# cv-stuttgart/PCFA

Measured on AMD Instinct MI355X. Metric: attack_steps_per_sec, higher is better.
Workload: dtype f32; 1 GPU; RAFT, 1 synthetic 436x1024 pair per GPU (padded 440x1024), disjoint delta, change_of_variables, delta_bound=0.005, zero target, L-BFGS max_iter=10; weights=random:1234, parallelism=pairs sharded 1/GPU, closure_launch=hipGraph replay

## Files before the change

### include/pcfa_hip.h

```cpp
#ifndef PCFA_HIP_H
#define PCFA_HIP_H

#include <stddef.h>
#include <stdint.h>

#ifdef __cplusplus
extern "C" {
#endif

#define PCFA_OK 0
#define PCFA_ERR_INVALID_ARG (-1)
#define PCFA_ERR_UNSUPPORTED (-2)
#define PCFA_ERR_WORKSPACE (-3)

#if defined(__GNUC__)
#define PCFA_API __attribute__((visibility("default")))
#else
#define PCFA_API
#endif

#define PCFA_MAX_LEVELS 8
#define PCFA_ABI_VERSION 2

#define PCFA_LOSS_AEE 0
#define PCFA_LOSS_MSE 1
#define PCFA_LOSS_COSIM 2

#define PCFA_BOX_CLIPPING 0
#define PCFA_BOX_CHANGE_OF_VARIABLES 1

PCFA_API int pcfa_abi_version(void);
PCFA_API int pcfa_timing_arm(void* start_event, void* stop_event, int nth);

PCFA_API int pcfa_null_launch(void* stream);
PCFA_API int pcfa_poison_lds(unsigned pattern, void* stream);
PCFA_API int pcfa_peek_lds(unsigned* out, int n, void* stream);
PCFA_API long long pcfa_calib_mfma_f32(float* scratch, int blocks, int iters, void* stream);
PCFA_API int pcfa_calib_copy(const float* src, float* dst, long long n_floats, void* stream);
PCFA_API const char* pcfa_status_string(int status);


PCFA_API long long pcfa_corr_slab_floats(int H, int W, int num_levels);
PCFA_API long long pcfa_corr_level_offset(int H, int W, int num_levels, int level, int* h_l, int* w_l);

PCFA_API long long pcfa_corr_tiled_index(int H, int W, int num_levels, int level, int y, int x);

PCFA_API int pcfa_corr_f2ext_fwd(const float* fmap2, float* f2ext, int B, int D, int H, int W,
                        int num_levels, void* stream);

PCFA_API int pcfa_corr_pyramid_fwd(const float* fmap1, const float* f2ext, float* pyr, int B, int D,
                          int H, int W, int num_levels, void* stream);

PCFA_API size_t pcfa_corr_pyramid_bwd_workspace_bytes(int B, int D, int H, int W, int num_levels);
PCFA_API int pcfa_corr_pyramid_bwd(const float* dpyr, const float* fmap1, const float* f2ext,
                          float* dfmap1, float* dfmap2, void* workspace, size_t workspace_bytes,
                          int B, int D, int H, int W, int num_levels, void* stream);
PCFA_API size_t pcfa_corr_pyramid_bwd_windows_workspace_bytes(int B, int D, int H, int W, int num_levels);
PCFA_API int pcfa_corr_pyramid_bwd_windows(const float* dpyr, const float* fmap1, const float* f2ext, float* dfmap1,
                                  float* dfmap2, void* workspace, size_t workspace_bytes,
                                  const float* const* coords, int n_coords, int radius, int B, int D, int H, int W,
                                  int num_levels, void* stream);

PCFA_API int pcfa_corr_lookup_fwd(const float* pyr, const float* coords, float* out, int B, int H, int W,
                         int num_levels, int radius, void* stream);

PCFA_API int pcfa_corr_lookup_bwd(float* dpyr, const float* coords, const float* grad_out, int B, int H,
                         int W, int num_levels, int radius, void* stream);

PCFA_API size_t pcfa_corr_ondemand_workspace_bytes(int B, int D, int H, int W, int num_levels);
PCFA_API int pcfa_corr_ondemand_prepare(const float* fmap1, const float* fmap2, void* workspace, int B, int D, int H,
                               int W, int num_levels, void* stream);
PCFA_API int pcfa_corr_ondemand_fwd(const void* workspace, const float* coords, float* out, int B, int D, int H, int W,
                           int num_levels, int radius, void* stream);
PCFA_API int pcfa_corr_ondemand_bwd(void* workspace, const float* coords, const float* grad_out, int accumulate, int B,
                           int D, int H, int W, int num_levels, int radius, void* stream);
PCFA_API int pcfa_corr_ondemand_finish(const void* workspace, float* dfmap1, float* dfmap2, int B, int D, int H, int W,
                              int num_levels, void* stream);

PCFA_API int pcfa_corr_ondemand_fwd_tiled(const void* workspace, const float* coords, float* out, int B, int D, int H,
                                 int W, int num_levels, int radius, void* stream);
PCFA_API int pcfa_corr_ondemand_bwd_tiled(void* workspace, const float* coords, const float* grad_out, int accumulate,
                                 int B, int D, int H, int W, int num_levels, int radius, void* stream);
PCFA_API int pcfa_corr_ondemand_tile_geometry(int* tile_w, int* tile_h, int* max_positions);
PCFA_API int pcfa_corr_ondemand_tile_routes(const void* workspace, int B, int D, int H, int W, int num_levels,
                                   int* counts, void* stream);

PCFA_API size_t pcfa_gemm_f32_workspace_bytes(int M, int N, int batch, int splits);
PCFA_API int pcfa_gemm_f32(const float* A, const float* B, float* C, int M, int N, int K, long long lda, long long ldb,
                  long long ldc, int a_kmajor, int b_kmajor, int batch, long long bsA, long long bsB, long long bsC,
                  float alpha, int splits, void* workspace, size_t workspace_bytes, void* stream);
// ... 330 lines not shown
```

### pcfa_amd/_hip.py

```python
import ctypes
import os
from ctypes import c_char_p, c_double, c_float, c_int, c_longlong, c_size_t, c_uint, c_void_p, POINTER

ABI_VERSION = 2
LIB_PATH = os.environ.get("PCFA_HIP_LIB") or os.path.join(os.path.dirname(os.path.abspath(__file__)), "lib",
                                                          "libpcfa_hip.so")

PCFA_LOSS = {"aee": 0, "mse": 1, "cosim": 2}


class HipLibraryError(RuntimeError):
    pass


_P = c_void_p
_S4 = POINTER(c_longlong)

SIGNATURES = {
    "pcfa_abi_version": (c_int, []),
    "pcfa_timing_arm": (c_int, [_P, _P, c_int]),
    "pcfa_null_launch": (c_int, [_P]),
    "pcfa_poison_lds": (c_int, [c_uint, _P]),
    "pcfa_peek_lds": (c_int, [_P, c_int, _P]),
    "pcfa_calib_mfma_f32": (c_longlong, [_P, c_int, c_int, _P]),
    "pcfa_calib_copy": (c_int, [_P, _P, c_longlong, _P]),
    "pcfa_status_string": (c_char_p, [c_int]),
    "pcfa_corr_slab_floats": (c_longlong, [c_int, c_int, c_int]),
    "pcfa_corr_level_offset": (c_longlong, [c_int, c_int, c_int, c_int, POINTER(c_int), POINTER(c_int)]),
    "pcfa_corr_tiled_index": (c_longlong, [c_int, c_int, c_int, c_int, c_int, c_int]),
    "pcfa_corr_f2ext_fwd": (c_int, [_P, _P, c_int, c_int, c_int, c_int, c_int, _P]),
    "pcfa_corr_pyramid_fwd": (c_int, [_P, _P, _P, c_int, c_int, c_int, c_int, c_int, _P]),
    "pcfa_corr_pyramid_bwd_workspace_bytes": (c_size_t, [c_int, c_int, c_int, c_int, c_int]),
    "pcfa_corr_pyramid_bwd": (c_int, [_P, _P, _P, _P, _P, _P, c_size_t, c_int, c_int, c_int, c_int, c_int, _P]),
    "pcfa_corr_pyramid_bwd_windows_workspace_bytes": (c_size_t, [c_int, c_int, c_int, c_int, c_int]),
    "pcfa_corr_pyramid_bwd_windows": (c_int, [_P, _P, _P, _P, _P, _P, c_size_t, POINTER(c_void_p), c_int, c_int, c_int,
                                              c_int, c_int, c_int, c_int, _P]),
    "pcfa_corr_lookup_fwd": (c_int, [_P, _P, _P, c_int, c_int, c_int, c_int, c_int, _P]),
    "pcfa_corr_lookup_bwd": (c_int, [_P, _P, _P, c_int, c_int, c_int, c_int, c_int, _P]),
    "pcfa_corr_ondemand_workspace_bytes": (c_size_t, [c_int, c_int, c_int, c_int, c_int]),
    "pcfa_corr_ondemand_prepare": (c_int, [_P, _P, _P, c_int, c_int, c_int, c_int, c_int, _P]),
    "pcfa_corr_ondemand_fwd": (c_int, [_P, _P, _P, c_int, c_int, c_int, c_int, c_int, c_int, _P]),
    "pcfa_corr_ondemand_bwd": (c_int, [_P, _P, _P, c_int, c_int, c_int, c_int, c_int, c_int, c_int, _P]),
    "pcfa_corr_ondemand_finish": (c_int, [_P, _P, _P, c_int, c_int, c_int, c_int, c_int, _P]),
    "pcfa_corr_ondemand_fwd_tiled": (c_int, [_P, _P, _P, c_int, c_int, c_int, c_int, c_int, c_int, _P]),
    "pcfa_corr_ondemand_bwd_tiled": (c_int, [_P, _P, _P, c_int, c_int, c_int, c_int, c_int, c_int, c_int, _P]),
    "pcfa_corr_ondemand_tile_geometry": (c_int, [POINTER(c_int), POINTER(c_int), POINTER(c_int)]),
    "pcfa_corr_ondemand_tile_routes": (c_int, [_P, c_int, c_int, c_int, c_int, c_int, _P, _P]),
    "pcfa_gemm_f32_workspace_bytes": (c_size_t, [c_int, c_int, c_int, c_int]),
    "pcfa_gemm_f32": (c_int, [_P, _P, _P, c_int, c_int, c_int, c_longlong, c_longlong, c_longlong, c_int, c_int, c_int,
                              c_longlong, c_longlong, c_longlong, c_float, c_int, _P, c_size_t, _P]),
    "pcfa_gemm_bf16x3_workspace_bytes": (c_size_t, [c_int, c_int, c_int, c_int]),
    "pcfa_gemm_bf16x3": (c_int, [_P, _P, _P, c_int, c_int, c_int, c_longlong, c_longlong, c_longlong, c_int, c_int,
                                 c_int, c_longlong, c_longlong, c_longlong, c_float, c_int, _P, c_size_t, _P]),
    "pcfa_corr_pyramid_fwd_bf16x3": (c_int, [_P, _P, _P, c_int, c_int, c_int, c_int, c_int, _P]),
    "pcfa_softmax_rows_fwd": (c_int, [_P, _P, c_longlong, c_int, _P]),
    "pcfa_softmax_rows_bwd": (c_int, [_P, _P, _P, c_longlong, c_int, _P]),
    "pcfa_attn_stream_lse": (c_int, [_P, _P, _P, c_int, c_int, c_int, c_float, _P]),
    "pcfa_attn_stream_fwd": (c_int, [_P, _P, _P, _P, _P, c_int, c_int, c_int, c_float, _P]),
    "pcfa_attn_stream_dv": (c_int, [_P, _P, _P, _P, _P, c_int, c_int, c_int, c_float, _P]),
    "pcfa_attn_stream_delta": (c_int, [_P, _P, _P, c_longlong, c_int, c_int, _P]),
    "pcfa_attn_stream_dqk": (c_int, [_P, _P, _P, _P, _P, _P, _P, _P, c_int, c_int, c_int, c_int, c_float, _P]),
    "pcfa_lookup_convc1_packed_floats": (c_longlong, [c_int]),
    "pcfa_lookup_convc1_pack_weights": (c_int, [_P, _P, c_int, c_int, _P]),
    "pcfa_lookup_convc1_fwd": (c_int, [_P, _P, _P, _P, _P, c_int, c_int, c_int, c_int, c_int, c_int, c_int, _P]),
    "pcfa_lookup_convc1_bwd": (c_int, [_P, _P, _P, _P, _P, c_int, c_int, c_int, c_int, c_int, c_int, c_int, _P]),
    "pcfa_spatial_corr_out_size": (c_int, [c_int] * 10 + [POINTER(c_int), POINTER(c_int)]),
    "pcfa_spatial_corr_fwd": (c_int, [_P, _P, _P] + [c_int] * 16 + [_P]),
# ... 182 lines not shown
```

### pcfa_amd/csrc/corr_pyramid.hip

```cpp
#include "common.hpp"
#include "gemm_tile.hpp"

namespace {

#ifndef PCFA_GEMM_BK
#define PCFA_GEMM_BK 16
#endif
#ifndef PCFA_GEMM_STORE_MID
#define PCFA_GEMM_STORE_MID 0
#endif
#ifndef PCFA_GEMM_STORE_MID_AT
#define PCFA_GEMM_STORE_MID_AT 4
#endif
constexpr int BK = PCFA_GEMM_BK;
constexpr int NLD = BK / 8;
constexpr int KV = BK / 4;
constexpr int LDS_KM = 132;
constexpr int LDS_MK = 130;

template <bool KMAJ>
__device__ __forceinline__ void tile_load(const float* __restrict__ X, long long ld, int dim,
                                          int d0, int k0, int kend, bool vec, float4 (&r)[NLD]) {
  const int tid = threadIdx.x;
#pragma unroll
// ... 109 lines not shown
      row + (okY ? u.off1 + (((Y1 >> 2) * u.tw1 + (X1 >> 2)) << 4) + ((Y1 & 3) << 2) + (X1 & 3) : 0));
  const float d1a = (okY && X1 < u.w1) ? g1.x + 0.25f * d2 : 0.f;
  const float d1b = (okY && X1 + 1 < u.w1) ? g1.y + 0.25f * d2 : 0.f;
  v.x += 0.25f * d1a;
  v.y += 0.25f * d1a;
  v.z += 0.25f * d1b;
  v.w += 0.25f * d1b;
  return v;
}

template <bool KMAJ>
__device__ __forceinline__ void tile_load_unpool(const float* __restrict__ X, long long ld, int dim, int d0, int k0,
                                                 int kend, const UnpoolArgs& u, float4 (&r)[NLD]) {
  static_assert(BK % 16 == 0, "whole 4x4 tiles per stage and query");
  const int tid = threadIdx.x;
#pragma unroll
  for (int i = 0; i < NLD; ++i) {
    const int f = tid + 256 * i;
    int q, col;
    if (KMAJ) {
      q = min(k0 + f / 32, kend - 1);
      col = min(d0 + (f % 32) * 4, dim - 4);
    } else {
      q = min(d0 + f / KV, dim - 1);
      col = min(k0 + (f % KV) * 4, kend - 4);
    }
    const int T0 = col >> 4, y = (col & 15) >> 2;
    const int ty = T0 / u.tw0, tx = T0 - ty * u.tw0;
    const float* row = X + (long long)q * ld;
    r[i] = unpool_piece(row, *reinterpret_cast<const float4*>(row + col), ty, tx, y, u);
  }
}

constexpr int SEG_INTS = 10;
template <bool A_KM, bool B_KN, bool FAST, bool POOL, bool UNPOOL = false, bool SPARSE = false>
__device__ __forceinline__ void gemm_f32_mfma_body(
    const float* __restrict__ A, const float* __restrict__ B, float* __restrict__ C, int M,
    int N, int K, long long lda, long long ldb, long long ldc, long long bsA, long long bsB,
    long long bsC, int splits, int kchunk, long long ssC, float div, int vecA, int vecB, const PoolArgs& pool,
    const UnpoolArgs& unpool = UnpoolArgs{}, const int* __restrict__ segs = nullptr) {
  static_assert(!UNPOOL || FAST, "the un-pooling loader is the branch-free one");
  static_assert(!SPARSE || (FAST && !POOL && !UNPOOL), "segment lists ride on the branch-free loader");
  constexpr int SA = A_KM ? LDS_KM : LDS_MK;
  constexpr int SB = B_KN ? LDS_KM : LDS_MK;
  constexpr int STAGE = 2 * BK * SA + 2 * BK * SB;
  constexpr int LDSF = POOL && BM * SC > STAGE ? BM * SC : STAGE;
  __shared__ __attribute__((aligned(16))) float smem[LDSF];
  float (*sA)[BK * SA] = reinterpret_cast<float (*)[BK * SA]>(smem);
  float (*sB)[BK * SB] = reinterpret_cast<float (*)[BK * SB]>(smem + 2 * BK * SA);

  const int batch = blockIdx.z / splits;
  const int split = blockIdx.z - batch * splits;
  A += batch * bsA;
  B += batch * bsB;
  C += batch * bsC + split * ssC;
  int kbeg = split * kchunk;
  const int kend = SPARSE ? K : min(K, kbeg + kchunk);
  int by = blockIdx.y, bx = blockIdx.x;
  gemm_tile_xcd_order(by, bx);
  const int m0 = by * BM;
  int n0 = bx * BN;
  bool pooled = false;
  if (POOL) {
    if (bx < pool.nb0) {
      pooled = true;
      N = pool.S0;
    } else {
      n0 = pool.off_tail + (bx - pool.nb0) * BN;
    }
  }

  const int lane = threadIdx.x & 63, wave = threadIdx.x >> 6;
  const int wr = wave >> 1, wc = wave & 1;
  const int l31 = lane & 31, lh = lane >> 5;

  f32x16 acc[2][2];
#pragma unroll
  for (int i = 0; i < 2; ++i)
#pragma unroll
    for (int j = 0; j < 2; ++j)
#pragma unroll
      for (int r = 0; r < 16; ++r) acc[i][j][r] = 0.f;

  float4 ra[NLD], rb[NLD];
  int nk = (kend - kbeg + BK - 1) / BK;
  int sb[4] = {0, 0, 0, 0}, se[4] = {0, 0, 0, 0}, seg = 0;
  if (SPARSE) {
    const int* sg = segs + ((long long)batch * gridDim.x + bx) * SEG_INTS;
    int total = 0;
#pragma unroll
    for (int i = 0; i < 4; ++i) {
      sb[i] = sg[1 + 2 * i];
      se[i] = sg[2 + 2 * i];
      total += (se[i] - sb[i]) / BK;
    }
    const int t0 = (int)((long long)total * split / splits), t1 = (int)((long long)total * (split + 1) / splits);
    nk = t1 - t0;
    int rem = t0;
    while (seg < 3 && rem >= (se[seg] - sb[seg]) / BK) {
      rem -= (se[seg] - sb[seg]) / BK;
      ++seg;
    }
    kbeg = sb[seg] + rem * BK;
  }
  int kcur = kbeg;
  if (nk > 0) {
    if (FAST) {
      tile_load_fast<A_KM>(A, lda, M, m0, kbeg, kend, ra);
      if (UNPOOL) tile_load_unpool<B_KN>(B, ldb, N, n0, kbeg, kend, unpool, rb);
      else tile_load_fast<B_KN>(B, ldb, N, n0, kbeg, kend, rb);
      tile_mask<A_KM>(M, m0, kbeg, kend, ra);
      tile_mask<B_KN>(N, n0, kbeg, kend, rb);
    } else {
      tile_load<A_KM>(A, lda, M, m0, kbeg, kend, vecA, ra);
      tile_load<B_KN>(B, ldb, N, n0, kbeg, kend, vecB, rb);
    }
    tile_store<A_KM>(sA[0], ra);
    tile_store<B_KN>(sB[0], rb);
  }
  __syncthreads();
  int cur = 0;
  for (int kt = 0; kt < nk; ++kt) {
    const bool more = kt + 1 < nk;
    int k0 = kbeg + (kt + 1) * BK;
    if (SPARSE) {
      k0 = kcur + BK;
      if (k0 >= se[seg] && seg < 3 && se[seg + 1] > sb[seg + 1]) {
        ++seg;
        k0 = sb[seg];
      }
      kcur = k0;
    }
    if (FAST) {
      tile_load_fast<A_KM>(A, lda, M, m0, min(k0, kend - 4), kend, ra);
      if (UNPOOL) tile_load_unpool<B_KN>(B, ldb, N, n0, min(k0, kend - 4), kend, unpool, rb);
      else tile_load_fast<B_KN>(B, ldb, N, n0, min(k0, kend - 4), kend, rb);
      __builtin_amdgcn_sched_barrier(0);
    } else if (more) {
      tile_load<A_KM>(A, lda, M, m0, k0, kend, vecA, ra);
      tile_load<B_KN>(B, ldb, N, n0, k0, kend, vecB, rb);
    }
    const float* a = sA[cur] + wr * 64 + l31;
    const float* b = sB[cur] + wc * 64 + l31;
#pragma unroll
    for (int kk = 0; kk < BK; kk += 2) {
      const float a0 = a[(kk + lh) * SA], a1 = a[(kk + lh) * SA + 32];
      const float b0 = b[(kk + lh) * SB], b1 = b[(kk + lh) * SB + 32];
      acc[0][0] = __builtin_amdgcn_mfma_f32_32x32x2f32(a0, b0, acc[0][0], 0, 0, 0);
      acc[0][1] = __builtin_amdgcn_mfma_f32_32x32x2f32(a0, b1, acc[0][1], 0, 0, 0);
      acc[1][0] = __builtin_amdgcn_mfma_f32_32x32x2f32(a1, b0, acc[1][0], 0, 0, 0);
      acc[1][1] = __builtin_amdgcn_mfma_f32_32x32x2f32(a1, b1, acc[1][1], 0, 0, 0);
#if PCFA_GEMM_STORE_MID
      if (FAST && kk == PCFA_GEMM_STORE_MID_AT) {
        __builtin_amdgcn_sched_barrier(0);
        tile_mask<A_KM>(M, m0, k0, kend, ra);
        tile_mask<B_KN>(N, n0, k0, kend, rb);
        tile_store<A_KM>(sA[cur ^ 1], ra);
        tile_store<B_KN>(sB[cur ^ 1], rb);
        __builtin_amdgcn_sched_barrier(0);
      }
#endif
    }
// ... 109 lines not shown
  }
  for (int l = 1; l < P.L; ++l)
    for (int i = threadIdx.x; i < P.h[l] * P.w[l]; i += blockDim.x) {
      const int y = i / P.w[l], x = i - y * P.w[l];
      s_lv[loff[l] + i] = src[pcfa_tiled_index(P, l, y, x)];
    }
  __syncthreads();
  for (int l = P.L - 1; l >= 2; --l) {
    const int hl = P.h[l], wl = P.w[l], wp = P.w[l - 1];
    const float* g = s_lv + loff[l];
    float* gp = s_lv + loff[l - 1];
    for (int i = threadIdx.x; i < 4 * hl * wl; i += blockDim.x) {
      const int y = i / (2 * wl), x = i - y * (2 * wl);
      gp[y * wp + x] += g[(y >> 1) * wl + (x >> 1)] / 4.0f;
    }
    __syncthreads();
  }
  const int W0 = P.w[0];
  for (int i = threadIdx.x; i < Q; i += blockDim.x) {
    const int y = i / W0, x = i - y * W0;
    float v = src[pcfa_tiled_index(P, 0, y, x)];
    if (P.L > 1 && (y >> 1) < P.h[1] && (x >> 1) < P.w[1])
      v += s_lv[loff[1] + (y >> 1) * P.w[1] + (x >> 1)] / 4.0f;
    dst[i] = v;
  }
}

size_t pooled_lds_bytes(const PyrLayout& P) {
  size_t n = 4;
  for (int l = 1; l < P.L; ++l) n += (size_t)P.h[l] * P.w[l];
  return n * sizeof(float);
}

constexpr int BWD_SPLITS = 8;
constexpr int MAX_COORDS = 32;

struct CoordList {
  const float* p[MAX_COORDS];
  int n;
};

__global__ __launch_bounds__(256) void corr_window_rows_kernel(CoordList cl, int H, int W, int r, PyrLayout P,
                                                                int* __restrict__ rows) {
  __shared__ float s_lo[4], s_hi[4];
  const int b = blockIdx.y, qy = blockIdx.x, Q = H * W;
  float lo = 3.0e38f, hi = -3.0e38f;
  bool bad = false;
  for (int i = 0; i < cl.n; ++i) {
    const float* cy = cl.p[i] + ((long long)b * 2 + 1) * Q + (long long)qy * W;
    for (int x = threadIdx.x; x < W; x += blockDim.x) {
      const float v = cy[x];
      bad = bad || !(v == v);
      lo = fminf(lo, v);
      hi = fmaxf(hi, v);
    }
  }
  if (bad) { lo = -3.0e38f; hi = 3.0e38f; }
#pragma unroll
  for (int o = 32; o > 0; o >>= 1) {
    lo = fminf(lo, __shfl_xor(lo, o, 64));
    hi = fmaxf(hi, __shfl_xor(hi, o, 64));
  }
  if ((threadIdx.x & 63) == 0) {
    s_lo[threadIdx.x >> 6] = lo;
    s_hi[threadIdx.x >> 6] = hi;
  }
  __syncthreads();
  if (threadIdx.x < P.L) {
    const int l = threadIdx.x;
    lo = fminf(fminf(s_lo[0], s_lo[1]), fminf(s_lo[2], s_lo[3]));
    hi = fmaxf(fmaxf(s_hi[0], s_hi[1]), fmaxf(s_hi[2], s_hi[3]));
    const float inv = 1.0f / (float)(1 << l);
    const float flo = fminf(fmaxf(floorf(lo * inv), -1.0e8f), 1.0e8f), fhi = fminf(fmaxf(floorf(hi * inv), -1.0e8f), 1.0e8f);
    int* o = rows + (((long long)b * P.L + l) * H + qy) * 2;
    o[0] = max((int)flo - r - 1, 0);
    o[1] = min((int)fhi + r + 2, P.h[l] - 1);
  }
}

__global__ __launch_bounds__(256) void corr_window_segments_kernel(const int* __restrict__ rows, int H, int W, PyrLayout P,
                                                                    int nbA, int nbB, int* __restrict__ segA,
                                                                    int* __restrict__ segB) {
  const int b = blockIdx.y, Q = H * W;
  const int* s_rows = rows + (long long)b * P.L * H * 2;
  const int j0 = blockIdx.x * blockDim.x + threadIdx.x;
  if (j0 < nbA) {
    const int j = j0;
    const int qa = (j * BN) / W, qb = min((j * BN + BN - 1) / W, H - 1);
    int* o = segA + ((long long)b * nbA + j) * SEG_INTS;
    int n = 0;
    for (int l = 0; l < P.L; ++l) {
      int ylo = 1 << 30, yhi = -1;
      for (int qy = qa; qy <= qb; ++qy) {
        const int a = s_rows[(l * H + qy) * 2], c = s_rows[(l * H + qy) * 2 + 1];
        if (a <= c) { ylo = min(ylo, a); yhi = max(yhi, c); }
      }
      if (ylo <= yhi) {
        const int beg = P.off[l] + (ylo >> 2) * P.tw[l] * 16, end = P.off[l] + ((yhi >> 2) + 1) * P.tw[l] * 16;
        if (n > 0 && o[2 * n] == beg) o[2 * n] = end;
        else { o[1 + 2 * n] = beg; o[2 + 2 * n] = end; ++n; }
      }
    }
    o[0] = n;
    for (int i = n; i < 4; ++i) { o[1 + 2 * i] = 0; o[2 + 2 * i] = 0; }
    o[9] = 0;
  }
  if (j0 >= nbA && j0 < nbA + nbB) {
    const int j = j0 - nbA;
    const int ca = j * BN, cb = min(j * BN + BN, P.slab) - 1;
    int qlo = 1 << 30, qhi = -1;
    for (int l = 0; l < P.L; ++l) {
      const int lbeg = P.off[l], lend = (l + 1 < P.L ? P.off[l + 1] : P.zero) - 1;
      const int a = max(ca, lbeg), c = min(cb, lend);
      if (a > c) continue;
      const int ya = ((a - lbeg) / (P.tw[l] * 16)) * 4, yb = ((c - lbeg) / (P.tw[l] * 16)) * 4 + 3;
      for (int qy = 0; qy < H; ++qy) {
        const int ra = s_rows[(l * H + qy) * 2], rc = s_rows[(l * H + qy) * 2 + 1];
        if (ra <= rc && ra <= yb && rc >= ya) { qlo = min(qlo, qy); qhi = max(qhi, qy); }
      }
    }
    int* o = segB + ((long long)b * nbB + j) * SEG_INTS;
    for (int i = 0; i < SEG_INTS; ++i) o[i] = 0;
    if (qlo <= qhi) {
      o[0] = 1;
      o[1] = (qlo * W) / BK * BK;
      o[2] = min(((qhi + 1) * W + BK - 1) / BK * BK, (Q + BK - 1) / BK * BK);
    }
  }
}

int choose_kchunk(int K, int splits) {
  int per = (K + splits - 1) / splits;
  return ((per + BK - 1) / BK) * BK;
}

}

extern "C" long long pcfa_corr_slab_floats(int H, int W, int num_levels) {
  PyrLayout P;
  if (!pcfa_make_layout(P, H, W, num_levels)) return -1;
  return P.slab;
}

extern "C" long long pcfa_corr_level_offset(int H, int W, int num_levels, int level, int* h_l,
                                            int* w_l) {
  PyrLayout P;
  if (!pcfa_make_layout(P, H, W, num_levels) || level < 0 || level >= num_levels) return -1;
  if (h_l) *h_l = P.h[level];
  if (w_l) *w_l = P.w[level];
  return P.off[level];
}

extern "C" long long pcfa_corr_tiled_index(int H, int W, int num_levels, int level, int y, int x) {
  PyrLayout P;
  if (!pcfa_make_layout(P, H, W, num_levels) || level < 0 || level >= num_levels || y < 0 ||
      x < 0 || y >= P.h[level] || x >= P.w[level])
    return -1;
  return pcfa_tiled_index(P, level, y, x);
}

// ... 35 lines not shown
  dim3 grid(pcfa_cdiv(S, BN), pcfa_cdiv(Q, BM), B);
#define PCFA_GEMM_ARGS fmap1, f2ext, pyr, Q, S, D, (long long)Q, (long long)S, (long long)S, (long long)D * Q, \
                       (long long)D * S, (long long)Q * S, 1, ((D + BK - 1) / BK) * BK, 0LL, sqrtf((float)D), vecA, vecB
  if (vecA && vecB && D % 4 == 0 && Q >= 4)
    pcfa_launch(gemm_f32_mfma_kernel<true, true, true>, grid, dim3(256), 0, (hipStream_t)stream, PCFA_GEMM_ARGS);
  else
    pcfa_launch(gemm_f32_mfma_kernel<true, true, false>, grid, dim3(256), 0, (hipStream_t)stream, PCFA_GEMM_ARGS);
#undef PCFA_GEMM_ARGS
  PCFA_LAUNCH_CHECK();
  return PCFA_OK;
}

extern "C" size_t pcfa_corr_pyramid_bwd_workspace_bytes(int B, int D, int H, int W,
                                                        int num_levels) {
  PyrLayout P;
  if (B < 1 || D < 1 || !pcfa_make_layout(P, H, W, num_levels)) return 0;
  const size_t Q = (size_t)H * W, S = P.slab;
  return sizeof(float) * ((size_t)BWD_SPLITS * B * D * Q + (size_t)BWD_SPLITS * B * D * S +
                          (size_t)B * D * S);
}

static int pyramid_bwd(const float* dpyr, const float* fmap1, const float* f2ext, float* dfmap1, float* dfmap2,
                       void* workspace, size_t workspace_bytes, int B, int D, int H, int W, int num_levels, void* stream,
                       const int* segA, const int* segB);

extern "C" int pcfa_corr_pyramid_bwd(const float* dpyr, const float* fmap1, const float* f2ext,
                                     float* dfmap1, float* dfmap2, void* workspace,
                                     size_t workspace_bytes, int B, int D, int H, int W,
                                     int num_levels, void* stream) {
  return pyramid_bwd(dpyr, fmap1, f2ext, dfmap1, dfmap2, workspace, workspace_bytes, B, D, H, W, num_levels, stream,
                     nullptr, nullptr);
}

extern "C" size_t pcfa_corr_pyramid_bwd_windows_workspace_bytes(int B, int D, int H, int W, int num_levels) {
  PyrLayout P;
  const size_t base = pcfa_corr_pyramid_bwd_workspace_bytes(B, D, H, W, num_levels);
  if (base == 0 || !pcfa_make_layout(P, H, W, num_levels)) return 0;
  const size_t nbA = (size_t)pcfa_cdiv((long long)H * W, BN), nbB = (size_t)pcfa_cdiv(P.slab, BN);
  return ((base + 15) & ~(size_t)15) + sizeof(int) * (SEG_INTS * B * (nbA + nbB) + 2 * (size_t)B * P.L * H);
}

extern "C" int pcfa_corr_pyramid_bwd_windows(const float* dpyr, const float* fmap1, const float* f2ext, float* dfmap1,
                                             float* dfmap2, void* workspace, size_t workspace_bytes,
                                             const float* const* coords, int n_coords, int radius, int B, int D, int H,
                                             int W, int num_levels, void* stream) {
  PyrLayout P;
  if (!dpyr || !fmap1 || !f2ext || !dfmap1 || !dfmap2 || !workspace || B < 1 || D < 1 || radius < 0 ||
      !pcfa_make_layout(P, H, W, num_levels))
    return PCFA_ERR_INVALID_ARG;
  const size_t base = (pcfa_corr_pyramid_bwd_workspace_bytes(B, D, H, W, num_levels) + 15) & ~(size_t)15;
  const long long Q = (long long)H * W;
  const bool fast = Q % 4 == 0 && aligned16(f2ext) && aligned16(dpyr) && aligned16(fmap1) && Q >= 4;
  if (!coords || n_coords < 1 || n_coords > MAX_COORDS || !fast || H > 65535 || num_levels > 4)
    return pyramid_bwd(dpyr, fmap1, f2ext, dfmap1, dfmap2, workspace, workspace_bytes, B, D, H, W, num_levels, stream,
                       nullptr, nullptr);
  if (workspace_bytes < pcfa_corr_pyramid_bwd_windows_workspace_bytes(B, D, H, W, num_levels)) return PCFA_ERR_WORKSPACE;
  const int nbA = pcfa_cdiv(Q, BN), nbB = pcfa_cdiv(P.slab, BN);
  int* segA = reinterpret_cast<int*>((char*)workspace + base);
  int* segB = segA + (size_t)SEG_INTS * B * nbA;
  CoordList cl;
  cl.n = n_coords;
  for (int i = 0; i < MAX_COORDS; ++i) cl.p[i] = i < n_coords ? coords[i] : nullptr;
  for (int i = 0; i < n_coords; ++i)
    if (!cl.p[i]) return PCFA_ERR_INVALID_ARG;
  int* rows = segB + (size_t)SEG_INTS * B * nbB;
  pcfa_launch(corr_window_rows_kernel, dim3(H, B), dim3(256), 0, (hipStream_t)stream, cl, H, W, radius, P, rows);
  PCFA_LAUNCH_CHECK();
  pcfa_launch(corr_window_segments_kernel, dim3(pcfa_cdiv(nbA + nbB, 256), B), dim3(256), 0, (hipStream_t)stream,
              (const int*)rows, H, W, P, nbA, nbB, segA, segB);
  PCFA_LAUNCH_CHECK();
  return pyramid_bwd(dpyr, fmap1, f2ext, dfmap1, dfmap2, workspace, base, B, D, H, W, num_levels, stream, segA, segB);
}

static int pyramid_bwd(const float* dpyr, const float* fmap1, const float* f2ext, float* dfmap1, float* dfmap2,
                       void* workspace, size_t workspace_bytes, int B, int D, int H, int W, int num_levels, void* stream,
                       const int* segA, const int* segB) {
  PyrLayout P;
  if (!dpyr || !fmap1 || !f2ext || !dfmap1 || !dfmap2 || !workspace || B < 1 || D < 1 ||
      !pcfa_make_layout(P, H, W, num_levels))
    return PCFA_ERR_INVALID_ARG;
  if (workspace_bytes < pcfa_corr_pyramid_bwd_workspace_bytes(B, D, H, W, num_levels))
    return PCFA_ERR_WORKSPACE;
  hipStream_t s = (hipStream_t)stream;
  const int Q = H * W, S = P.slab;
  const float div = sqrtf((float)D);
  float* part1 = (float*)workspace;
  float* part2 = part1 + (size_t)BWD_SPLITS * B * D * Q;
  float* df2ext = part2 + (size_t)BWD_SPLITS * B * D * S;

  static const bool unpool_on = getenv("PCFA_PYRAMID_UNPOOL") && atoi(getenv("PCFA_PYRAMID_UNPOOL")) == 1;
  if (P.L == 4 && W % 16 == 0 && Q % 4 == 0 && aligned16(f2ext) && aligned16(dpyr) && aligned16(fmap1) && unpool_on) {
    UnpoolArgs ua;
    ua.tw0 = P.tw[0];
    ua.off1 = P.off[1]; ua.tw1 = P.tw[1]; ua.h1 = P.h[1]; ua.w1 = P.w[1];
    ua.off2 = P.off[2]; ua.tw2 = P.tw[2]; ua.h2 = P.h[2]; ua.w2 = P.w[2];
    ua.off3 = P.off[3]; ua.tw3 = P.tw[3]; ua.h3 = P.h[3]; ua.w3 = P.w[3];
    const int S0 = P.off[1];
    {
      const int kchunk = choose_kchunk(S0, BWD_SPLITS);
      dim3 grid(pcfa_cdiv(Q, BN), pcfa_cdiv(D, BM), B * BWD_SPLITS);
      pcfa_launch(corr_pyramid_unpool_gemm_kernel<false>, grid, dim3(256), 0, s, f2ext, dpyr, part1, D, Q, S0,
                  (long long)S, (long long)S, (long long)Q, (long long)D * S, (long long)Q * S, (long long)D * Q,
// ... 126 lines not shown
```

### pcfa_amd/ops/corr.py

```python
import ctypes
import os

import torch

from .. import _hip
from . import core
from .conv import FEWIN_SHAPES, _conv3x3_cat_fill, _conv3x3_packed, _conv3x3_run, conv_fewin
from .core import _call, _dev, _note_work, _pair, _ptr, _ptr_off, _stream, cached_pack


class _CorrState:
    __slots__ = ("B", "D", "H", "W", "L", "r", "slab", "pyr", "f2ext", "dpyr", "token_grad", "coords_bwd", "bwd_windows", "mfma")


class _CorrBuild(torch.autograd.Function):

    @staticmethod
    def forward(ctx, fmap1, fmap2, state):
        lib = _hip.load()
        B, D, H, W = fmap1.shape
        f1 = fmap1.contiguous()
        f2 = fmap2.contiguous()
        slab = state.slab
        state.f2ext = torch.empty((B, D, slab), device=f1.device, dtype=torch.float32)
        state.pyr = torch.empty((B * H * W, slab), device=f1.device, dtype=torch.float32)
        _call("pcfa_corr_f2ext_fwd", _ptr(f2), _ptr(state.f2ext), B, D, H, W, state.L)
        _call("pcfa_corr_pyramid_fwd" if state.mfma == "f32" else "pcfa_corr_pyramid_fwd_bf16x3", _ptr(f1),
              _ptr(state.f2ext), _ptr(state.pyr), B, D, H, W, state.L)
        ctx.state = state
        ctx.save_for_backward(f1)
        return torch.zeros(1, device=f1.device, dtype=torch.float32)

    @staticmethod
    def backward(ctx, grad_token):
        st = ctx.state
        (f1,) = ctx.saved_tensors
        if st.dpyr is None:
            z = torch.zeros_like(f1)
            st.token_grad = None
            return z, z.clone(), None
        lib = _hip.load()
        B, D, H, W = st.B, st.D, st.H, st.W
        df1 = torch.empty_like(f1)
        df2 = torch.empty_like(f1)
        cs = st.coords_bwd if (st.coords_bwd and len(st.coords_bwd) <= 32 and st.bwd_windows and st.L <= 4) else []
        if cs:
            nbytes = lib.pcfa_corr_pyramid_bwd_windows_workspace_bytes(B, D, H, W, st.L)
            ws = torch.empty((nbytes + 3) // 4, device=f1.device, dtype=torch.float32)
            ptrs = (ctypes.c_void_p * len(cs))(*[c.data_ptr() for c in cs])
            _call("pcfa_corr_pyramid_bwd_windows", _ptr(st.dpyr), _ptr(f1), _ptr(st.f2ext), _ptr(df1), _ptr(df2), _ptr(ws),
                  ctypes.c_size_t(nbytes), ptrs, len(cs), st.r, B, D, H, W, st.L)
            if core.work_recorder() is not None:
                base = (int(lib.pcfa_corr_pyramid_bwd_workspace_bytes(B, D, H, W, st.L)) + 15) & ~15
                nbA, nbB = -(-(H * W) // 128), -(-st.slab // 128)
                seg = ws.view(torch.int32)[base // 4: base // 4 + 10 * B * (nbA + nbB)].cpu().view(-1, 10).long()
                live = torch.arange(4)[None, :] < seg[:, :1]
                k = ((seg[:, 2:9:2] - seg[:, 1:8:2]) * live).sum(1)
                dense = 2.0 * B * D * (H * W) ** 2
                _note_work("corr_pyramid_gemm_dfmap1", dense, 2.0 * D * 128 * float(k[:B * nbA].sum()))
                _note_work("corr_pyramid_gemm_df2ext", dense, 2.0 * D * 128 * float(k[B * nbA:].sum()))
        else:
            nbytes = lib.pcfa_corr_pyramid_bwd_workspace_bytes(B, D, H, W, st.L)
            ws = torch.empty((nbytes + 3) // 4, device=f1.device, dtype=torch.float32)
            _call("pcfa_corr_pyramid_bwd", _ptr(st.dpyr), _ptr(f1), _ptr(st.f2ext), _ptr(df1), _ptr(df2), _ptr(ws),
                  ctypes.c_size_t(nbytes), B, D, H, W, st.L)
        st.dpyr = None
        st.token_grad = None
        st.coords_bwd = None
        return df1, df2, None


def _token_grad(st, device):
    if st.token_grad is None:
        st.token_grad = torch.zeros(1, device=device, dtype=torch.float32)
        return st.token_grad
    return None


class _CorrLookup(torch.autograd.Function):
    @staticmethod
    def forward(ctx, token, coords, state):
        if coords.requires_grad and torch.is_grad_enabled():
            raise RuntimeError("CorrBlock lookup: coords.requires_grad is not supported (detach the coordinates, as "
                               "models/raft/raft.py:122-123 does)")
        lib = _hip.load()
        st = state
        c = coords.contiguous()
        n1 = 2 * st.r + 1
        out = torch.empty((st.B, st.L * n1 * n1, st.H, st.W), device=c.device, dtype=torch.float32)
        _call("pcfa_corr_lookup_fwd", _ptr(st.pyr), _ptr(c), _ptr(out), st.B, st.H, st.W, st.L, st.r)
        ctx.state = st
        ctx.save_for_backward(c)
        return out

    @staticmethod
    def backward(ctx, grad_out):
        st = ctx.state
        (c,) = ctx.saved_tensors
        lib = _hip.load()
        if st.dpyr is None:
            st.dpyr = torch.zeros_like(st.pyr)
            st.coords_bwd = []
# ... 331 lines not shown
```

Before: 7.792 attack_steps/s.

## Use per-row run windows to tighten sparse K segments in pyramid backward

Adds a run-level window pass that records, per 16-pixel run of each query row, the texel box touched by the correlation lookups. The df2ext GEMM then iterates only over the query-row segments that actually reach each output tile, with up to 48 segments per tile and coarser fallback modes when that capacity is exceeded. The sparse df2ext GEMM also schedules its blocks longest-first to balance uneven work. The goal is to skip more dead K range in the backward GEMMs, at the cost of an extra precompute kernel, a larger segment table and more complex split bookkeeping.

```diff
diff --git a/include/pcfa_hip.h b/include/pcfa_hip.h
--- a/include/pcfa_hip.h
+++ b/include/pcfa_hip.h
@@ -56,6 +56,7 @@
                           float* dfmap1, float* dfmap2, void* workspace, size_t workspace_bytes,
                           int B, int D, int H, int W, int num_levels, void* stream);
 PCFA_API size_t pcfa_corr_pyramid_bwd_windows_workspace_bytes(int B, int D, int H, int W, int num_levels);
+PCFA_API int pcfa_corr_pyramid_bwd_windows_tables(int H, int W, int num_levels, int* out);
 PCFA_API int pcfa_corr_pyramid_bwd_windows(const float* dpyr, const float* fmap1, const float* f2ext, float* dfmap1,
                                   float* dfmap2, void* workspace, size_t workspace_bytes,
                                   const float* const* coords, int n_coords, int radius, int B, int D, int H, int W,
diff --git a/pcfa_amd/_hip.py b/pcfa_amd/_hip.py
--- a/pcfa_amd/_hip.py
+++ b/pcfa_amd/_hip.py
@@ -33,6 +33,7 @@
     "pcfa_corr_pyramid_bwd_workspace_bytes": (c_size_t, [c_int, c_int, c_int, c_int, c_int]),
     "pcfa_corr_pyramid_bwd": (c_int, [_P, _P, _P, _P, _P, _P, c_size_t, c_int, c_int, c_int, c_int, c_int, _P]),
     "pcfa_corr_pyramid_bwd_windows_workspace_bytes": (c_size_t, [c_int, c_int, c_int, c_int, c_int]),
+    "pcfa_corr_pyramid_bwd_windows_tables": (c_int, [c_int, c_int, c_int, POINTER(c_int)]),
     "pcfa_corr_pyramid_bwd_windows": (c_int, [_P, _P, _P, _P, _P, _P, c_size_t, POINTER(c_void_p), c_int, c_int, c_int,
                                               c_int, c_int, c_int, c_int, _P]),
     "pcfa_corr_lookup_fwd": (c_int, [_P, _P, _P, c_int, c_int, c_int, c_int, c_int, _P]),
diff --git a/pcfa_amd/csrc/corr_pyramid.hip b/pcfa_amd/csrc/corr_pyramid.hip
--- a/pcfa_amd/csrc/corr_pyramid.hip
+++ b/pcfa_amd/csrc/corr_pyramid.hip
@@ -165,7 +165,18 @@
   }
 }
 
-constexpr int SEG_INTS = 10;
+constexpr int SEG_CAP = 48;
+constexpr int SEG_INTS = 4 + 2 * SEG_CAP;
+constexpr int RUN = 16;
+
+__device__ __forceinline__ void sparse_longest_first(int& by, int& bx, int& bz) {
+  const int nx = gridDim.x, ny = gridDim.y, nz = gridDim.z;
+  const int id = (blockIdx.z * ny + blockIdx.y) * nx + blockIdx.x, rest = id % (ny * nz);
+  bx = nx - 1 - id / (ny * nz);
+  by = rest / nz;
+  bz = rest - by * nz;
+}
+
 template <bool A_KM, bool B_KN, bool FAST, bool POOL, bool UNPOOL = false, bool SPARSE = false>
 __device__ __forceinline__ void gemm_f32_mfma_body(
     const float* __restrict__ A, const float* __restrict__ B, float* __restrict__ C, int M,
@@ -182,15 +193,16 @@
   float (*sA)[BK * SA] = reinterpret_cast<float (*)[BK * SA]>(smem);
   float (*sB)[BK * SB] = reinterpret_cast<float (*)[BK * SB]>(smem + 2 * BK * SA);
 
-  const int batch = blockIdx.z / splits;
-  const int split = blockIdx.z - batch * splits;
+  int by = blockIdx.y, bx = blockIdx.x, bz = blockIdx.z;
+  if (SPARSE && B_KN) sparse_longest_first(by, bx, bz);
+  else gemm_tile_xcd_order(by, bx);
+  const int batch = bz / splits;
+  const int split = bz - batch * splits;
   A += batch * bsA;
   B += batch * bsB;
   C += batch * bsC + split * ssC;
   int kbeg = split * kchunk;
   const int kend = SPARSE ? K : min(K, kbeg + kchunk);
-  int by = blockIdx.y, bx = blockIdx.x;
-  gemm_tile_xcd_order(by, bx);
   const int m0 = by * BM;
   int n0 = bx * BN;
   bool pooled = false;
@@ -217,24 +229,42 @@
 
   float4 ra[NLD], rb[NLD];
   int nk = (kend - kbeg + BK - 1) / BK;
-  int sb[4] = {0, 0, 0, 0}, se[4] = {0, 0, 0, 0}, seg = 0;
+  const int* sg = nullptr;
+  int nseg = 0, seg = 0, send = 0;
   if (SPARSE) {
-    const int* sg = segs + ((long long)batch * gridDim.x + bx) * SEG_INTS;
-    int total = 0;
-#pragma unroll
-    for (int i = 0; i < 4; ++i) {
-      sb[i] = sg[1 + 2 * i];
-      se[i] = sg[2 + 2 * i];
-      total += (se[i] - sb[i]) / BK;
-    }
-    const int t0 = (int)((long long)total * split / splits), t1 = (int)((long long)total * (split + 1) / splits);
-    nk = t1 - t0;
-    int rem = t0;
-    while (seg < 3 && rem >= (se[seg] - sb[seg]) / BK) {
-      rem -= (se[seg] - sb[seg]) / BK;
-      ++seg;
-    }
-    kbeg = sb[seg] + rem * BK;
+    sg = segs + ((long long)batch * gridDim.x + bx) * SEG_INTS;
+    nseg = min(sg[0], SEG_CAP);
+    if (!B_KN) {
+      int total = 0;
+      for (int i = 0; i < nseg; ++i) total += (sg[5 + 2 * i] - sg[4 + 2 * i]) / BK;
+      const int t0 = (int)((long long)total * split / splits), t1 = (int)((long long)total * (split + 1) / splits);
+      nk = t1 - t0;
+      if (nk > 0) {
+        int rem = t0, sbeg = sg[4];
+        send = sg[5];
+        while (seg + 1 < nseg && rem >= (send - sbeg) / BK) {
+          rem -= (send - sbeg) / BK;
+          ++seg;
+          sbeg = sg[4 + 2 * seg];
+          send = sg[5 + 2 * seg];
+        }
+        kbeg = sbeg + rem * BK;
+      }
+    } else {
+      const int total = (sg[3] - sg[2]) / BK;
+      const int kb0 = sg[2] + (int)((long long)total * split / splits) * BK;
+      const int kb1 = sg[2] + (int)((long long)total * (split + 1) / splits) * BK;
+      nk = 0;
+      for (int i = nseg - 1; i >= 0; --i) {
+        const int b = max(sg[4 + 2 * i], kb0), e = min(sg[5 + 2 * i], kb1);
+        if (e > b) {
+          nk += (e - b) / BK;
+          seg = i;
+          kbeg = b;
+          send = sg[5 + 2 * i];
+        }
+      }
+    }
   }
   int kcur = kbeg;
   if (nk > 0) {
@@ -258,9 +288,10 @@
     int k0 = kbeg + (kt + 1) * BK;
     if (SPARSE) {
       k0 = kcur + BK;
-      if (k0 >= se[seg] && seg < 3 && se[seg + 1] > sb[seg + 1]) {
+      if (k0 >= send && seg + 1 < nseg) {
         ++seg;
-        k0 = sb[seg];
+        k0 = sg[4 + 2 * seg];
+        send = sg[5 + 2 * seg];
       }
       kcur = k0;
     }
@@ -436,7 +467,10 @@
   return n * sizeof(float);
 }
 
-constexpr int BWD_SPLITS = 8;
+#ifndef PCFA_PYRAMID_BWD_SPLITS
+#define PCFA_PYRAMID_BWD_SPLITS 8
+#endif
+constexpr int BWD_SPLITS = PCFA_PYRAMID_BWD_SPLITS;
 constexpr int MAX_COORDS = 32;
 
 struct CoordList {
@@ -482,54 +516,196 @@
   }
 }
 
+__device__ __forceinline__ void window_record_a(const int* __restrict__ s_rows, int j, int H, int W, const PyrLayout& P,
+                                                int* __restrict__ o) {
+  const int qa = (j * BN) / W, qb = min((j * BN + BN - 1) / W, H - 1);
+  int n = 0;
+  for (int l = 0; l < P.L; ++l) {
+    int ylo = 1 << 30, yhi = -1;
+    for (int qy = qa; qy <= qb; ++qy) {
+      const int a = s_rows[(l * H + qy) * 2], c = s_rows[(l * H + qy) * 2 + 1];
+      if (a <= c) { ylo = min(ylo, a); yhi = max(yhi, c); }
+    }
+    if (ylo <= yhi) {
+      const int beg = P.off[l] + (ylo >> 2) * P.tw[l] * 16, end = P.off[l] + ((yhi >> 2) + 1) * P.tw[l] * 16;
+      if (n > 0 && o[3 + 2 * n] == beg) o[3 + 2 * n] = end;
+      else { o[4 + 2 * n] = beg; o[5 + 2 * n] = end; ++n; }
+    }
+  }
+  o[0] = n;
+  o[1] = 0;
+  o[2] = o[3] = 0;
+}
+
+__device__ __forceinline__ bool window_row_reaches(const int* __restrict__ s_rows, int qy, int ca, int cb, int H,
+                                                   const PyrLayout& P) {
+  bool hit = false;
+  for (int l = 0; l < P.L; ++l) {
+    const int lbeg = P.off[l], lend = (l + 1 < P.L ? P.off[l + 1] : P.zero) - 1;
+    const int a = max(ca, lbeg), c = min(cb, lend);
+    if (a > c) continue;
+    const int ya = ((a - lbeg) / (P.tw[l] * 16)) * 4, yb = ((c - lbeg) / (P.tw[l] * 16)) * 4 + 3;
+    const int ra = s_rows[(l * H + qy) * 2], rc = s_rows[(l * H + qy) * 2 + 1];
+    hit = hit || (ra <= rc && ra <= yb && rc >= ya);
+  }
+  return hit;
+}
+
 __global__ __launch_bounds__(256) void corr_window_segments_kernel(const int* __restrict__ rows, int H, int W, PyrLayout P,
                                                                     int nbA, int nbB, int* __restrict__ segA,
                                                                     int* __restrict__ segB) {
   const int b = blockIdx.y, Q = H * W;
   const int* s_rows = rows + (long long)b * P.L * H * 2;
   const int j0 = blockIdx.x * blockDim.x + threadIdx.x;
-  if (j0 < nbA) {
-    const int j = j0;
-    const int qa = (j * BN) / W, qb = min((j * BN + BN - 1) / W, H - 1);
-    int* o = segA + ((long long)b * nbA + j) * SEG_INTS;
-    int n = 0;
-    for (int l = 0; l < P.L; ++l) {
-      int ylo = 1 << 30, yhi = -1;
-      for (int qy = qa; qy <= qb; ++qy) {
-        const int a = s_rows[(l * H + qy) * 2], c = s_rows[(l * H + qy) * 2 + 1];
-        if (a <= c) { ylo = min(ylo, a); yhi = max(yhi, c); }
-      }
-      if (ylo <= yhi) {
-        const int beg = P.off[l] + (ylo >> 2) * P.tw[l] * 16, end = P.off[l] + ((yhi >> 2) + 1) * P.tw[l] * 16;
-        if (n > 0 && o[2 * n] == beg) o[2 * n] = end;
-        else { o[1 + 2 * n] = beg; o[2 + 2 * n] = end; ++n; }
-      }
-    }
-    o[0] = n;
-    for (int i = n; i < 4; ++i) { o[1 + 2 * i] = 0; o[2 + 2 * i] = 0; }
-    o[9] = 0;
-  }
+  if (j0 < nbA) window_record_a(s_rows, j0, H, W, P, segA + ((long long)b * nbA + j0) * SEG_INTS);
   if (j0 >= nbA && j0 < nbA + nbB) {
     const int j = j0 - nbA;
     const int ca = j * BN, cb = min(j * BN + BN, P.slab) - 1;
     int qlo = 1 << 30, qhi = -1;
-    for (int l = 0; l < P.L; ++l) {
-      const int lbeg = P.off[l], lend = (l + 1 < P.L ? P.off[l + 1] : P.zero) - 1;
-      const int a = max(ca, lbeg), c = min(cb, lend);
-      if (a > c) continue;
-      const int ya = ((a - lbeg) / (P.tw[l] * 16)) * 4, yb = ((c - lbeg) / (P.tw[l] * 16)) * 4 + 3;
+    for (int qy = 0; qy < H; ++qy)
+      if (window_row_reaches(s_rows, qy, ca, cb, H, P)) { qlo = min(qlo, qy); qhi = max(qhi, qy); }
+    int* o = segB + ((long long)b * nbB + j) * SEG_INTS;
+    o[0] = qlo <= qhi ? 1 : 0;
+    o[1] = 2;
+    o[2] = o[4] = qlo <= qhi ? (qlo * W) / BK * BK : 0;
+    o[3] = o[5] = qlo <= qhi ? min(((qhi + 1) * W + BK - 1) / BK * BK, (Q + BK - 1) / BK * BK) : 0;
+  }
+}
+
+__global__ __launch_bounds__(256) void corr_window_runs_kernel(CoordList cl, int H, int W, int r, PyrLayout P,
+                                                                int* __restrict__ rows, int* __restrict__ runs) {
+  __shared__ float s_lo[4], s_hi[4];
+  const int b = blockIdx.y, qy = blockIdx.x, Q = H * W, NR = W / RUN;
+  float rlo = 3.0e38f, rhi = -3.0e38f;
+  bool rbad = false;
+  for (int x0 = 0; x0 < W; x0 += 256) {
+    const int x = x0 + threadIdx.x;
+    float xlo = 3.0e38f, xhi = -3.0e38f, ylo = 3.0e38f, yhi = -3.0e38f;
+    bool bad = false;
+    if (x < W)
+      for (int i = 0; i < cl.n; ++i) {
+        const float* c = cl.p[i] + (long long)b * 2 * Q + (long long)qy * W + x;
+        const float vx = c[0], vy = c[Q];
+        bad = bad || !(vx == vx) || !(vy == vy);
+        rbad = rbad || !(vy == vy);
+        xlo = fminf(xlo, vx);
+        xhi = fmaxf(xhi, vx);
+        ylo = fminf(ylo, vy);
+        yhi = fmaxf(yhi, vy);
+      }
+    rlo = fminf(rlo, ylo);
+    rhi = fmaxf(rhi, yhi);
+#pragma unroll
+    for (int o = RUN / 2; o > 0; o >>= 1) {
+      xlo = fminf(xlo, __shfl_xor(xlo, o, 64));
+      xhi = fmaxf(xhi, __shfl_xor(xhi, o, 64));
+      ylo = fminf(ylo, __shfl_xor(ylo, o, 64));
+      yhi = fmaxf(yhi, __shfl_xor(yhi, o, 64));
+      bad = __shfl_xor((int)bad, o, 64) != 0 || bad;
+    }
+    if (bad) { xlo = ylo = -3.0e38f; xhi = yhi = 3.0e38f; }
+    if (x < W && x % RUN == 0)
+      for (int l = 0; l < P.L; ++l) {
+        const float inv = 1.0f / (float)(1 << l);
+        const auto tex = [&](float v) { return (int)fminf(fmaxf(floorf(v * inv), -1.0e8f), 1.0e8f); };
+        int4 t;
+        t.x = max(tex(xlo) - r - 1, 0);
+        t.y = min(tex(xhi) + r + 2, P.w[l] - 1);
+        t.z = max(tex(ylo) - r - 1, 0);
+        t.w = min(tex(yhi) + r + 2, P.h[l] - 1);
+        *reinterpret_cast<int4*>(runs + ((((long long)b * P.L + l) * H + qy) * NR + x / RUN) * 4) = t;
+      }
+  }
+  if (__syncthreads_or(rbad)) { rlo = -3.0e38f; rhi = 3.0e38f; }
+#pragma unroll
+  for (int o = 32; o > 0; o >>= 1) {
+    rlo = fminf(rlo, __shfl_xor(rlo, o, 64));
+    rhi = fmaxf(rhi, __shfl_xor(rhi, o, 64));
+  }
+  if ((threadIdx.x & 63) == 0) {
+    s_lo[threadIdx.x >> 6] = rlo;
+    s_hi[threadIdx.x >> 6] = rhi;
+  }
+  __syncthreads();
+  if (threadIdx.x < P.L) {
+    const int l = threadIdx.x;
+    rlo = fminf(fminf(s_lo[0], s_lo[1]), fminf(s_lo[2], s_lo[3]));
+    rhi = fmaxf(fmaxf(s_hi[0], s_hi[1]), fmaxf(s_hi[2], s_hi[3]));
+    const float inv = 1.0f / (float)(1 << l);
+    const float flo = fminf(fmaxf(floorf(rlo * inv), -1.0e8f), 1.0e8f), fhi = fminf(fmaxf(floorf(rhi * inv), -1.0e8f), 1.0e8f);
+    int* o = rows + (((long long)b * P.L + l) * H + qy) * 2;
+    o[0] = max((int)flo - r - 1, 0);
+    o[1] = min((int)fhi + r + 2, P.h[l] - 1);
+  }
+}
+
+constexpr int RUNS_MAX_H = 1024;
+__global__ __launch_bounds__(64) void corr_window_run_segments_kernel(const int* __restrict__ rows,
+                                                                       const int* __restrict__ runs, int H, int W,
+                                                                       PyrLayout P, int nbA, int nbB,
+                                                                       int* __restrict__ segA, int* __restrict__ segB) {
+  __shared__ short s_lo[RUNS_MAX_H], s_hi[RUNS_MAX_H];
+  const int b = blockIdx.y, NR = W / RUN, lane = threadIdx.x, Q = H * W;
+  const int* s_rows = rows + (long long)b * P.L * H * 2;
+  const int4* s_runs = reinterpret_cast<const int4*>(runs) + (long long)b * P.L * H * NR;
+  if ((int)blockIdx.x < nbA) {
+    if (lane == 0) window_record_a(s_rows, blockIdx.x, H, W, P, segA + ((long long)b * nbA + blockIdx.x) * SEG_INTS);
+    return;
+  }
+  const int j = blockIdx.x - nbA;
+  if (j >= nbB) return;
+  const int ca = j * BN, cb = min(j * BN + BN, P.slab) - 1;
+  for (int qy = lane; qy < H; qy += 64) {
+    int lo = NR, hi = -1;
+    const bool in_hull = window_row_reaches(s_rows, qy, ca, cb, H, P);
+    if (in_hull)
+      for (int l = 0; l < P.L; ++l) {
+        const int lbeg = P.off[l], lend = (l + 1 < P.L ? P.off[l + 1] : P.zero) - 1;
+        const int a = max(ca, lbeg), c = min(cb, lend);
+        if (a > c) continue;
+        const int ta = (a - lbeg) >> 4, tb = (c - lbeg) >> 4, tya = ta / P.tw[l], tyb = tb / P.tw[l];
+        const int txa = tya == tyb ? ta - tya * P.tw[l] : 0, txb = tya == tyb ? tb - tyb * P.tw[l] : P.tw[l] - 1;
+        for (int rx = 0; rx < NR; ++rx) {
+          const int4 v = s_runs[((long long)l * H + qy) * NR + rx];
+          if (v.x <= v.y && v.z <= v.w && v.x <= txb * 4 + 3 && v.y >= txa * 4 && v.z <= tyb * 4 + 3 && v.w >= tya * 4) {
+            lo = min(lo, rx);
+            hi = max(hi, rx);
+          }
+        }
+      }
+    s_lo[qy] = (short)lo;
+    s_hi[qy] = (short)(in_hull ? hi : -2);
+  }
+  __syncthreads();
+  if (lane == 0) {
+    int* o = segB + ((long long)b * nbB + j) * SEG_INTS;
+    int qlo = 1 << 30, qhi = -1;
+    for (int qy = 0; qy < H; ++qy)
+      if (s_hi[qy] != -2) { qlo = min(qlo, qy); qhi = max(qhi, qy); }
+    o[2] = qlo <= qhi ? (qlo * W) / BK * BK : 0;
+    o[3] = qlo <= qhi ? min(((qhi + 1) * W + BK - 1) / BK * BK, (Q + BK - 1) / BK * BK) : 0;
+    int n = 0, mode = 0;
+    for (; mode < 3; ++mode) {
+      n = 0;
+      int last = -1;
+      bool fits = true;
       for (int qy = 0; qy < H; ++qy) {
-        const int ra = s_rows[(l * H + qy) * 2], rc = s_rows[(l * H + qy) * 2 + 1];
-        if (ra <= rc && ra <= yb && rc >= ya) { qlo = min(qlo, qy); qhi = max(qhi, qy); }
+        if (s_hi[qy] < 0) continue;
+        const int beg = qy * W + (mode == 0 ? RUN * s_lo[qy] : 0), end = qy * W + (mode == 0 ? RUN * (s_hi[qy] + 1) : W);
+        if (n > 0 && (last == beg || mode == 2)) {
+          o[3 + 2 * n] = end;
+        } else {
+          if (n == SEG_CAP) { fits = false; break; }
+          o[4 + 2 * n] = beg;
+          o[5 + 2 * n] = end;
+          ++n;
+        }
+        last = end;
       }
-    }
-    int* o = segB + ((long long)b * nbB + j) * SEG_INTS;
-    for (int i = 0; i < SEG_INTS; ++i) o[i] = 0;
-    if (qlo <= qhi) {
-      o[0] = 1;
-      o[1] = (qlo * W) / BK * BK;
-      o[2] = min(((qhi + 1) * W + BK - 1) / BK * BK, (Q + BK - 1) / BK * BK);
-    }
+      if (fits) break;
+    }
+    o[0] = n;
+    o[1] = mode;
   }
 }
 
@@ -631,12 +807,41 @@
                      nullptr, nullptr);
 }
 
+struct WindowTables {
+  bool runs;
+  int nbA, nbB;
+  size_t rows_off;
+  size_t runs_off;
+  size_t ints;
+};
+static WindowTables window_tables(int B, int H, int W, const PyrLayout& P) {
+  WindowTables t;
+  t.runs = W % RUN == 0 && H <= RUNS_MAX_H && P.L <= 4;
+  t.nbA = pcfa_cdiv((long long)H * W, BN);
+  t.nbB = pcfa_cdiv(P.slab, BN);
+  t.rows_off = (size_t)SEG_INTS * B * (t.nbA + t.nbB);
+  t.runs_off = (t.rows_off + 2 * (size_t)B * P.L * H + 3) & ~(size_t)3;
+  t.ints = t.runs_off + (t.runs ? 4 * (size_t)B * P.L * H * (W / RUN) : 0);
+  return t;
+}
+
 extern "C" size_t pcfa_corr_pyramid_bwd_windows_workspace_bytes(int B, int D, int H, int W, int num_levels) {
   PyrLayout P;
   const size_t base = pcfa_corr_pyramid_bwd_workspace_bytes(B, D, H, W, num_levels);
   if (base == 0 || !pcfa_make_layout(P, H, W, num_levels)) return 0;
-  const size_t nbA = (size_t)pcfa_cdiv((long long)H * W, BN), nbB = (size_t)pcfa_cdiv(P.slab, BN);
-  return ((base + 15) & ~(size_t)15) + sizeof(int) * (SEG_INTS * B * (nbA + nbB) + 2 * (size_t)B * P.L * H);
+  return ((base + 15) & ~(size_t)15) + sizeof(int) * window_tables(B, H, W, P).ints;
+}
+
+extern "C" int pcfa_corr_pyramid_bwd_windows_tables(int H, int W, int num_levels, int* out) {
+  PyrLayout P;
+  if (!out || !pcfa_make_layout(P, H, W, num_levels)) return PCFA_ERR_INVALID_ARG;
+  const WindowTables t = window_tables(1, H, W, P);
+  out[0] = SEG_INTS;
+  out[1] = t.nbA;
+  out[2] = t.nbB;
+  out[3] = t.runs ? RUN : 0;
+  out[4] = SEG_CAP;
+  return PCFA_OK;
 }
 
 extern "C" int pcfa_corr_pyramid_bwd_windows(const float* dpyr, const float* fmap1, const float* f2ext, float* dfmap1,
@@ -654,7 +859,8 @@
     return pyramid_bwd(dpyr, fmap1, f2ext, dfmap1, dfmap2, workspace, workspace_bytes, B, D, H, W, num_levels, stream,
                        nullptr, nullptr);
   if (workspace_bytes < pcfa_corr_pyramid_bwd_windows_workspace_bytes(B, D, H, W, num_levels)) return PCFA_ERR_WORKSPACE;
-  const int nbA = pcfa_cdiv(Q, BN), nbB = pcfa_cdiv(P.slab, BN);
+  const WindowTables t = window_tables(B, H, W, P);
+  const int nbA = t.nbA, nbB = t.nbB;
   int* segA = reinterpret_cast<int*>((char*)workspace + base);
   int* segB = segA + (size_t)SEG_INTS * B * nbA;
   CoordList cl;
@@ -662,11 +868,19 @@
   for (int i = 0; i < MAX_COORDS; ++i) cl.p[i] = i < n_coords ? coords[i] : nullptr;
   for (int i = 0; i < n_coords; ++i)
     if (!cl.p[i]) return PCFA_ERR_INVALID_ARG;
-  int* rows = segB + (size_t)SEG_INTS * B * nbB;
-  pcfa_launch(corr_window_rows_kernel, dim3(H, B), dim3(256), 0, (hipStream_t)stream, cl, H, W, radius, P, rows);
-  PCFA_LAUNCH_CHECK();
-  pcfa_launch(corr_window_segments_kernel, dim3(pcfa_cdiv(nbA + nbB, 256), B), dim3(256), 0, (hipStream_t)stream,
-              (const int*)rows, H, W, P, nbA, nbB, segA, segB);
+  int* rows = segA + t.rows_off;
+  int* runs = segA + t.runs_off;
+  if (t.runs) {
+    pcfa_launch(corr_window_runs_kernel, dim3(H, B), dim3(256), 0, (hipStream_t)stream, cl, H, W, radius, P, rows, runs);
+    PCFA_LAUNCH_CHECK();
+    pcfa_launch(corr_window_run_segments_kernel, dim3(nbA + nbB, B), dim3(64), 0, (hipStream_t)stream, (const int*)rows,
+                (const int*)runs, H, W, P, nbA, nbB, segA, segB);
+  } else {
+    pcfa_launch(corr_window_rows_kernel, dim3(H, B), dim3(256), 0, (hipStream_t)stream, cl, H, W, radius, P, rows);
+    PCFA_LAUNCH_CHECK();
+    pcfa_launch(corr_window_segments_kernel, dim3(pcfa_cdiv(nbA + nbB, 256), B), dim3(256), 0, (hipStream_t)stream,
+                (const int*)rows, H, W, P, nbA, nbB, segA, segB);
+  }
   PCFA_LAUNCH_CHECK();
   return pyramid_bwd(dpyr, fmap1, f2ext, dfmap1, dfmap2, workspace, base, B, D, H, W, num_levels, stream, segA, segB);
 }
diff --git a/pcfa_amd/ops/corr.py b/pcfa_amd/ops/corr.py
--- a/pcfa_amd/ops/corr.py
+++ b/pcfa_amd/ops/corr.py
@@ -51,11 +51,9 @@
             _call("pcfa_corr_pyramid_bwd_windows", _ptr(st.dpyr), _ptr(f1), _ptr(st.f2ext), _ptr(df1), _ptr(df2), _ptr(ws),
                   ctypes.c_size_t(nbytes), ptrs, len(cs), st.r, B, D, H, W, st.L)
             if core.work_recorder() is not None:
-                base = (int(lib.pcfa_corr_pyramid_bwd_workspace_bytes(B, D, H, W, st.L)) + 15) & ~15
-                nbA, nbB = -(-(H * W) // 128), -(-st.slab // 128)
-                seg = ws.view(torch.int32)[base // 4: base // 4 + 10 * B * (nbA + nbB)].cpu().view(-1, 10).long()
-                live = torch.arange(4)[None, :] < seg[:, :1]
-                k = ((seg[:, 2:9:2] - seg[:, 1:8:2]) * live).sum(1)
+                seg, nbA, _ = window_segment_tables(ws, B, D, H, W, st.L)
+                live = torch.arange((seg.shape[1] - 4) // 2)[None, :] < seg[:, :1]
+                k = ((seg[:, 5::2] - seg[:, 4::2]) * live).sum(1)
                 dense = 2.0 * B * D * (H * W) ** 2
                 _note_work("corr_pyramid_gemm_dfmap1", dense, 2.0 * D * 128 * float(k[:B * nbA].sum()))
                 _note_work("corr_pyramid_gemm_df2ext", dense, 2.0 * D * 128 * float(k[B * nbA:].sum()))
@@ -68,6 +66,17 @@
         st.token_grad = None
         st.coords_bwd = None
         return df1, df2, None
+
+
+def window_segment_tables(ws, B, D, H, W, L):
+    lib = _hip.load()
+    info = (ctypes.c_int * 8)()
+    if lib.pcfa_corr_pyramid_bwd_windows_tables(H, W, L, info) != 0:
+        raise ValueError("no pyramid layout for %dx%d, %d levels" % (H, W, L))
+    rec, nbA, nbB = info[0], info[1], info[2]
+    base = (int(lib.pcfa_corr_pyramid_bwd_workspace_bytes(B, D, H, W, L)) + 15) & ~15
+    seg = ws.view(torch.int32)[base // 4: base // 4 + rec * B * (nbA + nbB)].cpu().view(-1, rec).long()
+    return seg, nbA, list(info)
 
 
 def _token_grad(st, device):
```

After: 7.885 attack_steps/s (median of 6 runs). 1.01x the previous value.
